# Maaz77/Head-Pose-Estimation-Model

Hardware: AMD Instinct MI355X
Metric: images/sec (train+infer) on 96×96 feature maps; yaw/pitch/roll MAE vs ref (higher is better)
Workload: dtype fp32; 1 GPU; Model-96 create_model(num_filters=360, dropout=0, l2=0.1) training, legacy Adam lr 2.8e-4, 96x96 feature maps (configs[3] per GPU: 512 images per rank); global_batch=512, per_gpu_batch=512, positions_per_image=9216, channels=96, parallelism=dp1

## Files before the change

### head-pose-estimation-model_amd/csrc/hpe_mlp2.hip

```cpp
#include <hip/hip_runtime.h>
#include <stdint.h>
#include <stdlib.h>

#include "hpe_common.h"
#include "hpe_dev.h"

#ifdef MLP2_BIG
#define MLP2_NS mlp2_big
#else
#define MLP2_NS mlp2_small
#endif
#define MLP2_BIG_ROWS (1 << 15)
namespace MLP2_NS {

#define MLP2_MAXW 12
#ifndef MLP2_BAR1_SKIP
#define MLP2_BAR1_SKIP 1
#endif
#ifndef MLP2_W88
#define MLP2_W88 2
#endif
#define MLP2_XS 100
#define MLP2_XF (32 * MLP2_XS)
#define MLP2_LAB 128
#define MLP2_RED 32
#define MLP2_FS 104
#define MLP2_TS 40
#define MLP2_A1W (15 * 68 + 64)
#define MLP2_PRE_HALVES (3 * 32 * MLP2_FS + 2 * 3 * 96 * MLP2_TS)

struct E2 {
  int act, drop;
  uint32_t thr;
  float keep;
};

struct TileImg {
  int img0, rem0, P;
  template <bool P32 = false>
  __device__ __forceinline__ int of(int r) const {
    const int t = rem0 + r;
    if (P32) return img0 + (t >= P ? 1 : 0);
    return img0 + (P >= 32 ? (t >= P ? 1 : 0) : (P == 1 ? t : t / P));
  }
  __device__ __forceinline__ void advance(int dq, int dr) {
    img0 += dq;
    rem0 += dr;
    if (rem0 >= P) { rem0 -= P; ++img0; }
  }
};

__device__ __forceinline__ float e_fwd(const E2& e, uint64_t seed, int64_t img, int ch, float z) {
  float a = act_f(e.act, z);
  if (e.drop >= 0) a = drop_hash(seed, e.drop, (uint64_t)img, ch) >= e.thr ? a / e.keep : 0.f;
  return a;
}

__device__ __forceinline__ float e_bwd(const E2& e, uint64_t seed, int64_t img, int ch, float g, float val) {
  if (e.drop >= 0) {
    if (drop_hash(seed, e.drop, (uint64_t)img, ch) < e.thr) return 0.f;
    g = g / e.keep;
    val = val * e.keep;
  }
  return e.act == ACT_LINEAR ? g : g * act_grad(e.act, val, 0.f);
}

__device__ __forceinline__ void stage_tile(const Args& args, float* xs, float* lab, int64_t row0,
                                           const TileImg& ti, int wave, int NCB, int lane, int Cin,
                                           bool labels, int XS = MLP2_XS) {
  const int64_t rem = args.nrows - 1 - row0;
  const int last = rem < 31 ? (int)rem : 31;
  const int P = args.P;
  const int q = Cin >> 2;
  if (!args.idx && P >= 32) {
    if (labels && wave == 0) {
#pragma unroll
      for (int pc = 0; pc < 2; ++pc) {
        const int slot = pc * 64 + lane;
        const int r = min(slot >> 2, last), j = min(slot & 3, 2);
        glds4(args.ytrue + (int64_t)ti.of(r) * 3 + j, lds_addr(lab + pc * 64));
      }
    }
    for (int r = wave; r < 32; r += NCB) {
      const int64_t srow = row0 + min(r, last);
      if (lane < q) glds16(args.x + srow * Cin + 4 * lane, lds_addr(xs + r * XS));
    }
    return;
  }
  const int lr = min(lane & 31, last);
  const int limg = ti.of(lr);
  const int lpos = (int)(row0 + lr - (int64_t)limg * P);
  const int lsrc = args.idx ? args.idx[limg] : limg;
  __builtin_amdgcn_s_waitcnt(0x0F70);
  if (labels && wave == 0) {
#pragma unroll
    for (int pc = 0; pc < 2; ++pc) {
      const int slot = pc * 64 + lane;
      const int r = min(slot >> 2, last), j = min(slot & 3, 2);
      const int64_t src = __shfl(lsrc, r, 64);
      glds4(args.ytrue + src * 3 + j, lds_addr(lab + pc * 64));
    }
  }
  for (int r = wave; r < 32; r += NCB) {
    const int rr = min(r, last);
    const int64_t srow = (int64_t)__builtin_amdgcn_readlane(lsrc, rr) * P +
                         __builtin_amdgcn_readlane(lpos, rr);
    if (lane < q) glds16(args.x + srow * Cin + 4 * lane, lds_addr(xs + r * XS));
  }
}

__device__ __forceinline__ int lane_now() {
  int l;
  asm volatile("v_mbcnt_lo_u32_b32 %0, -1, 0\n\tv_mbcnt_hi_u32_b32 %0, -1, %0" : "=v"(l));
  return l;
}

__device__ __forceinline__ void stage_contig(const Args& args, float* xs, float* lab, const float* tp,
                                             int64_t row0, const TileImg& ti, int wave, int NCB, int Cin,
                                             bool labels) {
  const int lane = lane_now();
  const int64_t rem = args.nrows - 1 - row0;
  const int last = rem < 31 ? (int)rem : 31;
  if (labels && wave == 0) {
    const float* yp = args.ytrue + (int64_t)ti.img0 * 3;
#pragma unroll
    for (int pc = 0; pc < 2; ++pc) {
      const int slot = pc * 64 + lane;
      const int r = min(slot >> 2, last), j = min(slot & 3, 2);
      glds4(yp + (ti.rem0 + r >= ti.P ? 3 + j : j), lds_addr(lab + pc * 64));
    }
  }
  const int q = Cin >> 2;
  for (int r = wave; r < 32; r += NCB)
    if (lane < q) glds16(tp + min(r, last) * Cin + 4 * lane, lds_addr(xs + r * MLP2_XS));
}

typedef _Float16 h4 __attribute__((ext_vector_type(4)));

__device__ __forceinline__ void split_d4(f32x4 v, h4& ch, h4& cl, h4& h) {
  const f32x4 s = v * SPLIT_C;
  ch = __builtin_convertvector(s, h4);
  cl = __builtin_convertvector(s - __builtin_convertvector(ch, f32x4), h4);
  h = __builtin_convertvector(v, h4);
}
__device__ __forceinline__ constexpr int a1_row(int g) { return 68 * (g ^ ((g >> 1) & 4)); }
#define MLP2_X_LIMIT (65520.f / SPLIT_C)
template <int KH>
__device__ __forceinline__ bool presplit_tile(const float* xs, _Float16* xf, _Float16* xt, int tid, int NT) {
  bool out = false;
  for (int i = tid; i < 32 * 24; i += NT) {
    const int r = i / 24, rem = i - r * 24, h = rem >= 12 ? 1 : 0, m0 = 4 * (rem - 12 * h);
    const f32x4 v = m0 < KH ? *(const f32x4*)(xs + r * MLP2_XS + KH * h + m0) : f32x4{0.f, 0.f, 0.f, 0.f};
    out |= !(fabsf(v.x) < MLP2_X_LIMIT) | !(fabsf(v.y) < MLP2_X_LIMIT) | !(fabsf(v.z) < MLP2_X_LIMIT) |
           !(fabsf(v.w) < MLP2_X_LIMIT);
    h4 ch, cl, hh;
    split_d4(v, ch, cl, hh);
    _Float16* d = xf + r * MLP2_FS + 48 * h + m0;
    *(h4*)(d) = ch;
    *(h4*)(d + 32 * MLP2_FS) = cl;
    *(h4*)(d + 64 * MLP2_FS) = hh;
  }
  for (int i = tid; i < 96 * 8; i += NT) {
    const int rg = i / 96, k = i - rg * 96, r = 4 * rg;
    const f32x4 v = {xs[r * MLP2_XS + k], xs[(r + 1) * MLP2_XS + k], xs[(r + 2) * MLP2_XS + k],
                     xs[(r + 3) * MLP2_XS + k]};
    const int p = (r & ~12) | ((r & 4) << 1) | ((r & 8) >> 1);
    h4 ch, cl, hh;
    split_d4(v, ch, cl, hh);
    _Float16* d = xt + k * MLP2_TS + p;
    *(h4*)(d) = ch;
    *(h4*)(d + 96 * MLP2_TS) = cl;
    *(h4*)(d + 192 * MLP2_TS) = hh;
  }
  return out;
}

template <int KH, int ACT1, bool DROP, int NWM, bool SPLIT, bool CONTIG = false>
__global__ void __launch_bounds__(NWM * 64) __attribute__((amdgpu_waves_per_eu(NWM == MLP2_MAXW || ACT1 < 0 ? 1 : MLP2_W88, 8))) mlp2_kernel(Args args) {
  static_assert(!CONTIG || (SPLIT && NWM == MLP2_MAXW), "CONTIG is an instantiation of the pre-split kernel");
  if (!SPLIT && args.guard && __hip_atomic_load(args.guard, __ATOMIC_RELAXED, __HIP_MEMORY_SCOPE_AGENT) != args.epoch) return;
#ifdef MLP2_STAMPS
  const uint64_t rt0 = __builtin_amdgcn_s_memrealtime();
#endif
  extern __shared__ __attribute__((aligned(16))) float lds[];
  constexpr int NKB = (2 * KH + 31) / 32;
  constexpr int T = 32;
  constexpr bool PRE = SPLIT && NWM == MLP2_MAXW;
  constexpr int NXB = PRE ? 1 : 2;
  constexpr bool LEAN = PRE && ACT1 >= 0;
  constexpr bool PAD1 = true;
  constexpr int A1S = MLP2_A1W;
  constexpr int HS = NWM == MLP2_MAXW ? 4 : 3;
  const int* prog = args.prog;
  const int* o = prog + prog[H_OPS_OFF];
  const int mode = prog[H_MODE];
  const bool train = mode == MODE_TRAIN;
  const int Cin = o[O_K], F = o[O_N], NCB = o[O_MODE];
  const int wave = __builtin_amdgcn_readfirstlane(threadIdx.x >> 6);
  const int lane = threadIdx.x & 63, half = lane >> 5, l32 = lane & 31;
  const int NT = blockDim.x;
  const int n = wave * 32 + l32;
  const bool nok = n < F;
  const int NPR = NWM == MLP2_MAXW ? MLP2_MAXW : NCB;
  float* xbuf = lds;
  float* lbuf = xbuf + NXB * MLP2_XF;
  float* part = lbuf + 2 * MLP2_LAB;
  float* dz2 = part + NPR * T * 4;
  float* a1s = dz2 + T * 4;
  float* w2t = a1s + NCB * A1S;
  float* b2t = w2t + NCB * 128;
  float* hacc = b2t + 4;
  float* red = hacc + NCB * 64 * HS;
  float* colt = red + MLP2_RED;
  _Float16* xfb = (_Float16*)(colt + NCB * 128);
  _Float16* xtb = xfb + 3 * 32 * MLP2_FS;

  E2 e1 = {o[O_EACT], o[O_EDROP], (uint32_t)o[O_ETHR], __int_as_float(o[O_EKEEP])};
  E2 e2 = {o[O_AUX2], o[O_TBASE], (uint32_t)o[O_TCOUNT], __int_as_float(o[O_F0])};
  const float inv_keep1 = 1.f / e1.keep;
  const float* W1 = args.params + o[O_W];
  const float* W2 = args.params + o[O_AUX0];

  const int64_t nrows = args.nrows;
  const int64_t ntiles = (nrows + T - 1) / T;
  const int P = args.P;
  const bool labels = mode != MODE_FWD;
  const int S = gridDim.x * T, dq = S / P, dr = S - dq * P;
  TileImg ti;
  ti.P = P;
  ti.img0 = (int)(blockIdx.x * T / P);
  ti.rem0 = (int)(blockIdx.x * T - ti.img0 * P);
  const float* xnext = CONTIG ? args.x + (int64_t)blockIdx.x * T * Cin : nullptr;
  const int64_t xstep = CONTIG ? (int64_t)gridDim.x * T * Cin : 0;
  if (blockIdx.x < ntiles) {
    if constexpr (CONTIG) stage_contig(args, xbuf, lbuf, xnext, (int64_t)blockIdx.x * T, ti, wave, NCB, Cin, labels);
    else stage_tile(args, xbuf, lbuf, (int64_t)blockIdx.x * T, ti, wave, NCB, lane, Cin, labels);
  }
  xnext += xstep;
  const int nc = min(n, F - 1);
  const float w2a = W2[nc * 3], w2b = W2[nc * 3 + 1], w2c = W2[nc * 3 + 2];
  const int o_bias = __builtin_amdgcn_readfirstlane(o[O_BIAS]), o_aux1 = __builtin_amdgcn_readfirstlane(o[O_AUX1]);
  const float b1r = args.params[max(o_bias, 0) + nc];
  float w2r[2];
#pragma unroll
  for (int t = 0; t < 2; ++t) {
    const int i = threadIdx.x + t * NT, nn = i >> 2, j = i & 3;
    w2r[t] = W2[min(nn, F - 1) * 3 + min(j, 2)];
  }
  const float b2r = args.params[max(o_aux1, 0) + min((int)threadIdx.x & 3, 2)];

  float wreg[SPLIT ? 1 : KH];
  SplitW wsp[SPLIT ? 6 : 1];
  float inv1 = 1.f, s2 = 1.f;
  bool wbad = false;
  if constexpr (SPLIT) {
    f32x8 v[6];
#pragma unroll
    for (int s = 0; s < 6; ++s) {
#pragma unroll
      for (int j = 0; j < 8; ++j) {
        const int k = half * KH + 8 * s + j;
        v[s][j] = 8 * s + j < KH ? W1[(size_t)min(k, Cin - 1) * F + nc] : 0.f;
      }
    }
    __builtin_amdgcn_sched_barrier(0);
    float mx = 0.f;
#pragma unroll
    for (int s = 0; s < 6; ++s) {
#pragma unroll
      for (int j = 0; j < 8; ++j) {
        const int k = half * KH + 8 * s + j;
        v[s][j] = (k < Cin && nok) ? v[s][j] : 0.f;
        mx = fmaxf(mx, fabsf(v[s][j]));
      }
    }
    mx = fmaxf(mx, __shfl_xor(mx, 32, 64));
    const float s1 = pow2_scale(mx, 13);
    inv1 = SPLIT_INV_C / s1;
#pragma unroll
    for (int s = 0; s < 6; ++s) {
      const f32x8 vs = v[s] * s1;
      wsp[s] = split_w8(vs);
      if (PRE) {
#pragma unroll
        for (int j = 0; j < 8; ++j) wbad |= !(fabsf(vs[j]) < 65520.f);
      }
    }
    s2 = pow2_scale(nok ? fmaxf(fmaxf(fabsf(w2a), fabsf(w2b)), fabsf(w2c)) : 0.f, 2);
  } else {
#pragma unroll
    for (int m = 0; m < KH; ++m) {
      const int k = half * KH + m;
      const float wv = W1[(size_t)min(k, Cin - 1) * F + nc];
      wreg[m] = (k < Cin && nok) ? wv : 0.f;
    }
  }
  bool bad = PRE && wbad && blockIdx.x < ntiles;
  {
    const float b1 = (nok && o_bias >= 0) ? b1r : 0.f;
    if (half == 0) *(f32x4*)(colt + n * 4) = f32x4{inv1, b1, s2, 0.f};
  }
#pragma unroll
  for (int t = 0; t < 2; ++t) {
    const int i = threadIdx.x + t * NT, nn = i >> 2, j = i & 3;
    if (i < NCB * 128) w2t[i] = (nn < F && j < 3) ? w2r[t] : 0.f;
  }
  if (threadIdx.x < 4) b2t[threadIdx.x] = (threadIdx.x < 3 && o_aux1 >= 0) ? b2r : 0.f;
  for (int i = threadIdx.x; i < NT * HS; i += NT) hacc[i] = 0.f;

  f32x16 dw[NKB];
#pragma unroll
  for (int s = 0; s < NKB; ++s) dw[s] = f32x16{};
  float dw2[3] = {0.f, 0.f, 0.f};
  float db1 = 0.f;

  const int NT3 = (NT / 3) * 3;

  for (int i = threadIdx.x; i < NXB * 32 * 16; i += NT) {
    const int r = i >> 4, c = Cin + (i & 15);
    if (c < 96) xbuf[r * MLP2_XS + c] = 0.f;
  }
  for (int i = NCB * T * 4 + threadIdx.x; i < NPR * T * 4; i += NT) part[i] = 0.f;
  __syncthreads();
  if constexpr (PRE) {
    asm volatile("s_waitcnt vmcnt(0)" ::: "memory");
    bar_lds();
    const bool xbad = presplit_tile<KH>(xbuf, xfb, xtb, threadIdx.x, NT);
    bad |= xbad && blockIdx.x < ntiles;
  }
  int buf = 0;
#ifdef MLP2_STAMPS
  uint32_t ph[9] = {};
  uint64_t tprev = __builtin_amdgcn_s_memtime();
  const uint64_t rt1 = __builtin_amdgcn_s_memrealtime();
#define STAMP(i) do { const uint64_t t_ = __builtin_amdgcn_s_memtime(); ph[i] += (uint32_t)(t_ - tprev); tprev = t_; } while (0)
#else
#define STAMP(i) do {} while (0)
#endif
  for (int tile = blockIdx.x; tile < (int)ntiles; tile += gridDim.x, buf ^= 1, ti.advance(dq, dr)) {
    const int tlane = PRE ? lane_now() : lane, thalf = tlane >> 5, tl32 = tlane & 31;
    const int tcol = wave * 32 + tl32;
    const bool tok = tcol < F;
    const int64_t row0 = (int64_t)tile * T;
    const float* xs = xbuf + (PRE ? 0 : buf) * MLP2_XF;
    const float* lab = lbuf + buf * MLP2_LAB;
    if constexpr (!PRE) asm volatile("s_waitcnt vmcnt(0)" ::: "memory");
    STAMP(0);
    if (!(MLP2_BAR1_SKIP && PRE && NCB >= 4 && tile != (int)blockIdx.x)) bar_lds();
    STAMP(1);
    if (tile + gridDim.x < ntiles) {
      TileImg tn = ti;
      tn.advance(dq, dr);
      if constexpr (CONTIG) {
        stage_contig(args, xbuf, lbuf + (buf ^ 1) * MLP2_LAB, xnext, (int64_t)(tile + gridDim.x) * T, tn,
                     wave, NCB, Cin, labels);
        xnext += xstep;
      } else {
        stage_tile(args, xbuf + (PRE ? 0 : (buf ^ 1)) * MLP2_XF, lbuf + (buf ^ 1) * MLP2_LAB,
                   (int64_t)(tile + gridDim.x) * T, tn, wave, NCB, tlane, Cin, labels);
      }
    }

    STAMP(2);
    uint32_t dmask = 0;
    {
      const float* ap = xs + tl32 * MLP2_XS + thalf * KH;
      f32x16 acc = {};
      if constexpr (PRE) {
        const _Float16* fp = xfb + tl32 * MLP2_FS + 48 * thalf;
        auto frag = [&](int s) {
          return SplitD{*(const h8*)(fp + 8 * s), *(const h8*)(fp + 32 * MLP2_FS + 8 * s),
                        *(const h8*)(fp + 64 * MLP2_FS + 8 * s)};
        };
        SplitD xd = frag(0);
#pragma unroll
        for (int s = 0; s < 6; ++s) {
          SplitD xn = xd;
          if (s + 1 < 6) xn = frag(s + 1);
          __builtin_amdgcn_sched_barrier(0);
          acc = mfma3_dw(xd, wsp[s], acc);
          xd = xn;
        }
        STAMP(3);
      } else if constexpr (SPLIT) {
#pragma unroll
        for (int s = 0; s < 6; ++s) {
          const f32x4 a0 = *(const f32x4*)(ap + 8 * s), a1 = *(const f32x4*)(ap + 8 * s + 4);
          acc = mfma3_dw(split_d8(f32x8{a0.x, a0.y, a0.z, a0.w, a1.x, a1.y, a1.z, a1.w}), wsp[s], acc);
          __builtin_amdgcn_sched_barrier(0);
        }
        bad |= !(fabsf(sum16(acc)) <= 3.0e38f);
      } else {
        f32x4 an = *(const f32x4*)(ap);
#pragma unroll
        for (int m = 0; m < KH; m += 4) {
          const f32x4 a = an;
          if (m + 4 < KH) an = *(const f32x4*)(ap + m + 4);
          acc = __builtin_amdgcn_mfma_f32_32x32x2f32(a.x, wreg[m + 0], acc, 0, 0, 0);
          acc = __builtin_amdgcn_mfma_f32_32x32x2f32(a.y, wreg[m + 1], acc, 0, 0, 0);
          acc = __builtin_amdgcn_mfma_f32_32x32x2f32(a.z, wreg[m + 2], acc, 0, 0, 0);
          acc = __builtin_amdgcn_mfma_f32_32x32x2f32(a.w, wreg[m + 3], acc, 0, 0, 0);
          __builtin_amdgcn_sched_barrier(0);
        }
      }
      if (DROP) {
        if (CONTIG || P >= 32) {
          const bool k0 = drop_hash(args.seed, e1.drop, (uint64_t)(ti.img0 + args.img_off), tcol) >= e1.thr;
          const bool k1 = drop_hash(args.seed, e1.drop, (uint64_t)(ti.img0 + 1 + args.img_off), tcol) >= e1.thr;
#pragma unroll
          for (int g = 0; g < 16; ++g) {
            const int r = (g & 3) + 8 * (g >> 2) + 4 * thalf;
            dmask |= (ti.rem0 + r >= P ? k1 : k0) ? (1u << g) : 0u;
          }
        } else {
#pragma unroll
          for (int g = 0; g < 16; ++g) {
            const int r = (g & 3) + 8 * (g >> 2) + 4 * thalf;
            dmask |= drop_hash(args.seed, e1.drop, (uint64_t)(ti.of(r) + args.img_off), tcol) >= e1.thr
                         ? (1u << g) : 0u;
          }
        }
      }
      const f32x4 cs = *(const f32x4*)(colt + tcol * 4);
#pragma unroll
      for (int g = 0; g < 16; ++g) {
        float z = act1_f<ACT1, SPLIT>(e1.act, SPLIT ? fmaf(acc[g], cs.x, cs.y) : acc[g] + cs.y);
        if (DROP) z = (dmask >> g) & 1u ? z * inv_keep1 : 0.f;
        acc[g] = LEAN || tok ? z : 0.f;
      }
#pragma unroll
      for (int g = 0; g < 16; ++g) a1s[wave * A1S + (PAD1 ? a1_row(g) : 64 * g) + tlane] = acc[g];
      __builtin_amdgcn_fence(__ATOMIC_RELEASE, "wavefront");
      __builtin_amdgcn_wave_barrier();
      __builtin_amdgcn_fence(__ATOMIC_ACQUIRE, "wavefront");
      {
        const int r = tl32, hh = (r >> 2) & 1, gr = (r & 3) + 4 * (r >> 3);
        const float* ar = a1s + wave * A1S + (PAD1 ? a1_row(gr) : 64 * gr) + hh * 32 + 16 * thalf;
        const float* wr = w2t + (wave * 32 + 16 * thalf) * 4;
        float s0 = 0.f, s1 = 0.f, s2 = 0.f;
#pragma unroll
        for (int i = 0; i < 16; i += 4) {
          const f32x4 av = *(const f32x4*)(ar + i);
#pragma unroll
          for (int e = 0; e < 4; ++e) {
            const f32x4 w = *(const f32x4*)(wr + (i + e) * 4);
            s0 = fmaf(av[e], w.x, s0);
            s1 = fmaf(av[e], w.y, s1);
            s2 = fmaf(av[e], w.z, s2);
          }
        }
        s0 += __shfl_xor(s0, 32, 64);
        s1 += __shfl_xor(s1, 32, 64);
        s2 += __shfl_xor(s2, 32, 64);
        if (thalf == 0) *(f32x4*)(part + (wave * T + r) * 4) = f32x4{s0, s1, s2, 0.f};
      }
    }
    STAMP(4);
    const bool early = PRE && NCB >= 4;
    if (early) asm volatile("s_waitcnt vmcnt(0)" ::: "memory");
    bar_lds();
    STAMP(5);
    if constexpr (PRE) {
      if (early && wave >= 2 && tile + gridDim.x < ntiles)
        bad |= presplit_tile<KH>(xbuf, xfb, xtb + (buf ^ 1) * 3 * 96 * MLP2_TS, threadIdx.x - 128, NT - 128);
    }

    auto head_item = [&](int it) {
      const int r = it / 3, j = it - r * 3;
      const int64_t R = row0 + r;
      float z = b2t[j];
      float pv[MLP2_MAXW];
#pragma unroll
      for (int w = 0; w < MLP2_MAXW; ++w) pv[w] = NWM == MLP2_MAXW || w < NCB ? part[(w * T + r) * 4 + j] : 0.f;
      float lv = 0.f, ha0 = 0.f, ha1 = 0.f, ha2 = 0.f;
      if (mode != MODE_FWD) {
        lv = lab[r * 4 + j];
        ha0 = hacc[threadIdx.x * HS + 0];
        ha1 = hacc[threadIdx.x * HS + 1];
        ha2 = hacc[threadIdx.x * HS + 2];
      }
#pragma unroll
      for (int w = 0; w < MLP2_MAXW; ++w) z += pv[w];
      const bool d2 = ACT1 < 0 || __builtin_expect(e2.drop >= 0, 0);
      int64_t img = 0;
      bool k2 = true;
      if (d2) {
        img = ti.of<CONTIG>(r) + args.img_off;
        if (ACT1 >= 0) k2 = drop_hash(args.seed, e2.drop, (uint64_t)img, j) >= e2.thr;
      }
      const float p = ACT1 >= 0 ? (d2 ? (k2 ? z / e2.keep : 0.f) : z) : e_fwd(e2, args.seed, img, j, z);
      if (mode == MODE_FWD) {
        if (R < nrows) args.y[R * 3 + j] = p;
      } else {
        float g = 0.f;
        if (R < nrows) {
          const float err = p - lv;
          ha0 = fmaf(err, err, ha0);
          ha1 += fabsf(err);
          g = SPLIT ? 2.f * err : 2.f * err * args.inv_count;
        }
        if (train) {
          g = ACT1 >= 0 ? (d2 ? (k2 ? g / e2.keep : 0.f) : g) : e_bwd(e2, args.seed, img, j, g, p);
          dz2[r * 4 + j] = g;
          ha2 += g;
        }
        hacc[threadIdx.x * HS + 0] = ha0;
        hacc[threadIdx.x * HS + 1] = ha1;
        hacc[threadIdx.x * HS + 2] = ha2;
      }
    };
    if constexpr (NWM == MLP2_MAXW) {
      if (threadIdx.x < T * 3) head_item(threadIdx.x);
    } else {
      for (int it = threadIdx.x; it < T * 3 && threadIdx.x < NT3; it += NT3) head_item(it);
    }
    STAMP(6);
    if constexpr (PRE) {
      asm volatile("s_waitcnt vmcnt(0)" ::: "memory");
      bar_lds();
      STAMP(7);
      if (!early && tile + gridDim.x < ntiles) {
        bad |= presplit_tile<KH>(xbuf, xfb, xtb + (buf ^ 1) * 3 * 96 * MLP2_TS, threadIdx.x, NT);
      }
      if (!train) continue;
    } else {
      if (!train) continue;
      bar_lds();
    }

    STAMP(8);
    {
      const f32x4 w2r = *(const f32x4*)(w2t + tcol * 4);
      const float s2 = colt[tcol * 4 + 2];
      const f32x4 w2v = PRE ? f32x4{w2r.x * s2, w2r.y * s2, w2r.z * s2, 0.f} : w2r;
      auto dz_of = [&](int g) {
        const int r = (g & 3) + 8 * (g >> 2) + 4 * thalf;
        const f32x4 d = *(const f32x4*)(dz2 + r * 4);
        const float a = a1s[wave * A1S + (PAD1 ? a1_row(g) : 64 * g) + tlane];
        const float da = PRE ? fmaf(d.z, w2v.z, fmaf(d.x, w2v.x, d.y * w2v.y))
                             : d.x * w2v.x + d.y * w2v.y + d.z * w2v.z;
        float gz, av = a;
        if (DROP) {
          gz = (dmask >> g) & 1u ? da * inv_keep1 : 0.f;
          av = a * e1.keep;
        } else {
          gz = da;
        }
        {
#pragma clang fp contract(off)
          gz = LEAN || tok ? gz * act1_g<ACT1>(e1.act, av) : 0.f;
          db1 += gz;
        }
        dw2[0] = fmaf(a, d.x, dw2[0]);
        dw2[1] = fmaf(a, d.y, dw2[1]);
        dw2[2] = fmaf(a, d.z, dw2[2]);
        return gz;
      };
      if constexpr (PRE) {
        const _Float16* th = xtb + buf * 3 * 96 * MLP2_TS + tl32 * MLP2_TS + 8 * thalf;
        f32x8 dv0, dv1;
#pragma unroll
        for (int j = 0; j < 8; ++j) dv0[j] = dz_of(j);
        const SplitW d0 = split_w8(dv0);
        __builtin_amdgcn_sched_barrier(0);
#pragma unroll
        for (int kb = 0; kb < NKB; ++kb) {
          const _Float16* q = th + kb * 32 * MLP2_TS;
          dw[kb] = mfma3_dw(SplitD{*(const h8*)(q), *(const h8*)(q + 96 * MLP2_TS), *(const h8*)(q + 192 * MLP2_TS)}, d0, dw[kb]);
        }
#pragma unroll
        for (int j = 0; j < 8; ++j) dv1[j] = dz_of(8 + j);
        __builtin_amdgcn_sched_barrier(0);
        const SplitW d1 = split_w8(dv1);
#pragma unroll
        for (int kb = 0; kb < NKB; ++kb) {
          const _Float16* q = th + 16 + kb * 32 * MLP2_TS;
          dw[kb] = mfma3_dw(SplitD{*(const h8*)(q), *(const h8*)(q + 96 * MLP2_TS), *(const h8*)(q + 192 * MLP2_TS)}, d1, dw[kb]);
        }
      } else if constexpr (SPLIT) {
#pragma unroll
        for (int s = 0; s < 2; ++s) {
          f32x8 dv;
#pragma unroll
          for (int j = 0; j < 8; ++j) {
            dv[j] = dz_of(8 * s + j);
            if ((j & 3) == 3) __builtin_amdgcn_sched_barrier(0);
          }
          const SplitW dsp = split_w8(dv * s2);
#pragma unroll
          for (int kb = 0; kb < NKB; ++kb) {
            const float* xp = xs + (4 * thalf) * MLP2_XS + kb * 32 + tl32;
            f32x8 xv;
#pragma unroll
            for (int j = 0; j < 8; ++j) xv[j] = xp[(16 * s + 8 * (j >> 2) + (j & 3)) * MLP2_XS];
            dw[kb] = mfma3_dw(split_d8(xv), dsp, dw[kb]);
            __builtin_amdgcn_sched_barrier(0);
          }
        }
      } else {
        float dz1[16];
#pragma unroll
        for (int g = 0; g < 16; ++g) {
          dz1[g] = dz_of(g);
          if ((g & 3) == 3) __builtin_amdgcn_sched_barrier(0);
        }
#pragma unroll
        for (int kb = 0; kb < NKB; ++kb) {
          const float* xp = xs + (4 * thalf) * MLP2_XS + kb * 32 + tl32;
          f32x16 acc = dw[kb];
          auto xat = [&](int g) { return xp[((g & 3) + 8 * (g >> 2)) * MLP2_XS]; };
          float x0 = xat(0), x1 = xat(1);
#pragma unroll
          for (int g = 0; g < 16; ++g) {
            const float xv = x0;
            x0 = x1;
            if (g + 2 < 16) x1 = xat(g + 2);
            acc = __builtin_amdgcn_mfma_f32_32x32x2f32(xv, dz1[g], acc, 0, 0, 0);
            __builtin_amdgcn_sched_barrier(0);
          }
          dw[kb] = acc;
        }
      }
    }
  }

#ifdef MLP2_STAMPS
  const uint64_t rt2 = __builtin_amdgcn_s_memrealtime();
  uint64_t rtA = 0, rtB = 0;
  if (PRE && blockIdx.x == 0 && lane == 0 && (wave == 0 || wave == 5))
    printf("STAMP w%d bwd+tail %u bar1 %u stage %u fwdmfma %u act+part %u bar2 %u head %u bar3 %u presplit %u\n", wave,
           ph[0], ph[1], ph[2], ph[3], ph[4], ph[5], ph[6], ph[7], ph[8]);
#endif
  const int flane = PRE ? lane_now() : lane, fhalf = flane >> 5;
  const int fcol = wave * 32 + (flane & 31);
  const bool fok = fcol < F;
  if (mode == MODE_FWD) {
    if (SPLIT && bad) __hip_atomic_store(args.guard, args.epoch, __ATOMIC_RELAXED, __HIP_MEMORY_SCOPE_AGENT);
    return;
  }
  const int slab = prog[H_SLAB];
  const int npt = prog[H_NPARAMS_TRAIN];
  float* ws = args.ws + (size_t)blockIdx.x * slab;
  const float sc = SPLIT ? args.inv_count : 1.f;
  const int oW = __builtin_amdgcn_readfirstlane(o[O_W]), oB = __builtin_amdgcn_readfirstlane(o[O_BIAS]);
  const int oA0 = __builtin_amdgcn_readfirstlane(o[O_AUX0]), oA1 = __builtin_amdgcn_readfirstlane(o[O_AUX1]);
  __syncthreads();
  const float s2f = colt[fcol * 4 + 2];
  if (train) {
    const float scw = SPLIT ? sc * (SPLIT_INV_C / s2f) : sc;
    float chk = 0.f;
#pragma unroll
    for (int kb = 0; kb < NKB; ++kb) {
      if (SPLIT) chk += sum16(dw[kb]);
#pragma unroll
      for (int g = 0; g < 16; ++g) {
        const int k = kb * 32 + (g & 3) + 8 * (g >> 2) + 4 * fhalf;
        if (k < Cin && fok) ws[oW + (size_t)k * F + fcol] = dw[kb][g] * scw;
      }
    }
    if (SPLIT) bad |= (!LEAN || fok) && !(fabsf(chk) <= 3.0e38f);
    const float tb = (db1 + __shfl_xor(db1, 32, 64)) * (PRE ? 1.f / s2f : 1.f);
    float t2[3];
#pragma unroll
    for (int j = 0; j < 3; ++j) t2[j] = dw2[j] + __shfl_xor(dw2[j], 32, 64);
    if (fhalf == 0 && fok) {
      if (oB >= 0) ws[oB + fcol] = tb * sc;
#pragma unroll
      for (int j = 0; j < 3; ++j) ws[oA0 + fcol * 3 + j] = t2[j] * sc;
    }
#ifdef MLP2_STAMPS
    rtA = __builtin_amdgcn_s_memrealtime();
#endif
    if (oA1 >= 0) {
      for (int j = wave; j < 3; j += NT >> 6) {
        float s = 0.f;
        for (int i = j + 3 * flane; i < NT3; i += 192) s += hacc[i * HS + 2];
        s = wave_sum(s);
        if (flane == 0) ws[oA1 + j] = s * sc;
      }
    }
#ifdef MLP2_STAMPS
    rtB = __builtin_amdgcn_s_memrealtime();
#endif
    __syncthreads();
  }
#ifdef MLP2_STAMPS
  const uint64_t rtC = __builtin_amdgcn_s_memrealtime();
#endif
  if (SPLIT && bad) __hip_atomic_store(args.guard, args.epoch, __ATOMIC_RELAXED, __HIP_MEMORY_SCOPE_AGENT);
  const float a = wave_sum(hacc[threadIdx.x * HS + 0]), b = wave_sum(hacc[threadIdx.x * HS + 1]);
  if (flane == 0) { red[wave] = a; red[MLP2_MAXW + wave] = b; }
  __syncthreads();
  if (threadIdx.x == 0) {
    float s0 = 0.f, s1 = 0.f;
    const int nw = NT >> 6;
    for (int w = 0; w < nw; ++w) { s0 += red[w]; s1 += red[MLP2_MAXW + w]; }
    ws[npt] = s0;
    ws[npt + 1] = s1;
  }
#ifdef MLP2_STAMPS
  if (PRE && threadIdx.x == 0) {
    const uint64_t rt3 = __builtin_amdgcn_s_memrealtime();
    printf("RT wg %d t0 %llu pro %llu loop %llu flush %llu wstore %llu db2 %llu sync %llu tail %llu\n", (int)blockIdx.x, (unsigned long long)rt0,
           (unsigned long long)(rt1 - rt0), (unsigned long long)(rt2 - rt1), (unsigned long long)(rt3 - rt2),
           (unsigned long long)(rtA - rt2), (unsigned long long)(rtB - rtA), (unsigned long long)(rtC - rtB), (unsigned long long)(rt3 - rtC));
  }
#endif
}

#ifdef MLP2_BIG
#define MLP2R_NU 2
#define MLP2R_LDS_FLOATS (2 * MLP2_XF + 2 * MLP2_LAB + MLP2R_NU * MLP2_A1W + 32 * 4 + MLP2R_NU * 128 + 4)

template <int KH, int ACT1, bool DROP>
__global__ void __launch_bounds__(64) __attribute__((amdgpu_waves_per_eu(1, 1))) mlp2r_kernel(Args args) {
  extern __shared__ __attribute__((aligned(16))) float lds[];
  constexpr int NU = MLP2R_NU;
  constexpr int NKB = (2 * KH + 31) / 32;
  constexpr int T = 32;
  constexpr int XS = KH == 44 ? 88 : MLP2_XS;
  const int* prog = args.prog;
  const int* o = prog + prog[H_OPS_OFF];
  const int Cin = o[O_K], F = o[O_N];
  const int lane = threadIdx.x, half = lane >> 5, l32 = lane & 31;
  float* xbuf = lds;
  float* lbuf = xbuf + 2 * MLP2_XF;
  float* a1p = lbuf + 2 * MLP2_LAB;
  float* dz2 = a1p + NU * MLP2_A1W;
  float* w2t = dz2 + 32 * 4;
  float* b2t = w2t + NU * 128;
  const E2 e1 = {o[O_EACT], o[O_EDROP], (uint32_t)o[O_ETHR], __int_as_float(o[O_EKEEP])};
  const E2 e2 = {o[O_AUX2], o[O_TBASE], (uint32_t)o[O_TCOUNT], __int_as_float(o[O_F0])};
  const float inv_keep1 = 1.f / e1.keep, inv_keep2 = 1.f / e2.keep;
  const float* W1 = args.params + o[O_W];
  const float* W2 = args.params + o[O_AUX0];
  const int o_bias = __builtin_amdgcn_readfirstlane(o[O_BIAS]), o_aux1 = __builtin_amdgcn_readfirstlane(o[O_AUX1]);

  const int64_t nrows = args.nrows;
  const int64_t ntiles = (nrows + T - 1) / T;
  const int P = args.P;
  const int S = gridDim.x * T, dq = S / P, dr = S - dq * P;
  TileImg ti;
  ti.P = P;
  ti.img0 = (int)(blockIdx.x * T / P);
  ti.rem0 = (int)(blockIdx.x * T - ti.img0 * P);
  auto stage = [&](float* xd, float* ld, int64_t r0, const TileImg& t) {
    if (XS == 88 && !args.idx && P >= 32 && r0 + T <= nrows && Cin == 88) {
#pragma unroll
      for (int pc = 0; pc < 2; ++pc) {
        const int slot = pc * 64 + lane;
        glds4(args.ytrue + (int64_t)t.of(slot >> 2) * 3 + min(slot & 3, 2), lds_addr(ld + pc * 64));
      }
#pragma unroll
      for (int i = 0; i < 11; ++i) glds16(args.x + r0 * 88 + 256 * i + 4 * lane, lds_addr(xd + 256 * i));
    } else {
      stage_tile(args, xd, ld, r0, t, 0, 1, lane, Cin, true, XS);
    }
  };
  if (blockIdx.x < ntiles) stage(xbuf, lbuf, (int64_t)blockIdx.x * T, ti);

  SplitW wsp[NU][6];
  float inv1[NU], b1v[NU], s2[NU], nm[NU];
  f32x4 w2v[NU];
  bool nok[NU];
  {
    f32x8 v[NU][6];
    float w2r[NU][3], b1r[NU];
#pragma unroll
    for (int u = 0; u < NU; ++u) {
      const int n = 32 * u + l32, nc = min(n, F - 1);
      nok[u] = n < F;
      nm[u] = nok[u] ? 1.f : 0.f;
#pragma unroll
      for (int j = 0; j < 3; ++j) w2r[u][j] = W2[nc * 3 + j];
      b1r[u] = args.params[max(o_bias, 0) + nc];
#pragma unroll
      for (int s = 0; s < 6; ++s) {
#pragma unroll
        for (int j = 0; j < 8; ++j) {
          const int k = half * KH + 8 * s + j;
          v[u][s][j] = 8 * s + j < KH ? W1[(size_t)min(k, Cin - 1) * F + nc] : 0.f;
        }
      }
    }
    const float b2r = args.params[max(o_aux1, 0) + min(lane & 3, 2)];
    __builtin_amdgcn_sched_barrier(0);
#pragma unroll
    for (int u = 0; u < NU; ++u) {
      float mx = 0.f;
#pragma unroll
      for (int s = 0; s < 6; ++s) {
#pragma unroll
        for (int j = 0; j < 8; ++j) {
          const int k = half * KH + 8 * s + j;
          v[u][s][j] = (k < Cin && nok[u]) ? v[u][s][j] : 0.f;
          mx = fmaxf(mx, fabsf(v[u][s][j]));
        }
      }
      mx = fmaxf(mx, __shfl_xor(mx, 32, 64));
      const float s1 = pow2_scale(mx, 13);
      inv1[u] = SPLIT_INV_C / s1;
#pragma unroll
      for (int s = 0; s < 6; ++s) wsp[u][s] = split_w8(v[u][s] * s1);
      w2v[u] = nok[u] ? f32x4{w2r[u][0], w2r[u][1], w2r[u][2], 0.f} : f32x4{0.f, 0.f, 0.f, 0.f};
      s2[u] = pow2_scale(nok[u] ? fmaxf(fmaxf(fabsf(w2r[u][0]), fabsf(w2r[u][1])), fabsf(w2r[u][2])) : 0.f, 2);
      b1v[u] = (nok[u] && o_bias >= 0) ? b1r[u] : 0.f;
      if (half == 0) *(f32x4*)(w2t + (32 * u + l32) * 4) = w2v[u];
    }
    if (lane < 4) b2t[lane] = (lane < 3 && o_aux1 >= 0) ? b2r : 0.f;
  }
  if (XS == 88) {
    for (int i = lane; i < 2 * (MLP2_XF - 32 * 88); i += 64)
      xbuf[(i >= MLP2_XF - 32 * 88 ? MLP2_XF : 0) + 32 * 88 + i % (MLP2_XF - 32 * 88)] = 0.f;
  } else {
    for (int i = lane; i < 2 * 32 * 16; i += 64) {
      const int r = i >> 4, c = Cin + (i & 15);
      if (c < 96) xbuf[r * MLP2_XS + c] = 0.f;
    }
  }

  f32x16 dw[NU][NKB];
#pragma unroll
  for (int u = 0; u < NU; ++u)
#pragma unroll
    for (int kb = 0; kb < NKB; ++kb) dw[u][kb] = f32x16{};
  float dw2[NU][3], db1[NU];
#pragma unroll
  for (int u = 0; u < NU; ++u) { dw2[u][0] = dw2[u][1] = dw2[u][2] = 0.f; db1[u] = 0.f; }
  float sse = 0.f, sae = 0.f, db2[3] = {0.f, 0.f, 0.f};
  bool bad = false;

  int buf = 0;
#ifdef MLP2R_STAMPS
  uint32_t ph[7] = {};
  uint64_t tprev = __builtin_amdgcn_s_memtime();
#define RSTAMP(i) do { const uint64_t t_ = __builtin_amdgcn_s_memtime(); ph[i] += (uint32_t)(t_ - tprev); tprev = t_; } while (0)
#else
#define RSTAMP(i) do {} while (0)
#endif
  for (int64_t tile = blockIdx.x; tile < ntiles; tile += gridDim.x, buf ^= 1, ti.advance(dq, dr)) {
    const int64_t row0 = tile * T;
    RSTAMP(0);
    asm volatile("s_waitcnt vmcnt(0)" ::: "memory");
    if (tile + gridDim.x < ntiles) {
      TileImg tn = ti;
      tn.advance(dq, dr);
      stage(xbuf + (buf ^ 1) * MLP2_XF, lbuf + (buf ^ 1) * MLP2_LAB, (tile + gridDim.x) * T, tn);
    }
    const float* xs = xbuf + buf * MLP2_XF;
    const float* lab = lbuf + buf * MLP2_LAB;
    RSTAMP(1);

    f32x16 acc[NU];
#pragma unroll
    for (int u = 0; u < NU; ++u) acc[u] = f32x16{};
    {
      const float* ap = xs + l32 * XS + half * KH;
      f32x4 xa[12];
#pragma unroll
      for (int s = 0; s < 12; ++s) xa[s] = *(const f32x4*)(ap + 4 * s);
#pragma unroll
      for (int s = 0; s < 6; ++s) {
        const f32x4 a0 = xa[2 * s], a1 = xa[2 * s + 1];
        const SplitD xd = split_d8(f32x8{a0.x, a0.y, a0.z, a0.w, a1.x, a1.y, a1.z, a1.w});
#pragma unroll
        for (int u = 0; u < NU; ++u) acc[u] = mfma3_dw(xd, wsp[u][s], acc[u]);
      }
    }
    RSTAMP(2);
    uint32_t dmask[NU];
#pragma unroll
    for (int u = 0; u < NU; ++u) {
      bad |= !(fabsf(sum16(acc[u])) <= 3.0e38f);
      const int n = 32 * u + l32;
      dmask[u] = 0u;
      if (DROP) {
        if (P >= 32) {
          const bool k0 = drop_hash(args.seed, e1.drop, (uint64_t)(ti.img0 + args.img_off), n) >= e1.thr;
          const bool k1 = drop_hash(args.seed, e1.drop, (uint64_t)(ti.img0 + 1 + args.img_off), n) >= e1.thr;
#pragma unroll
          for (int g = 0; g < 16; ++g) {
            const int r = (g & 3) + 8 * (g >> 2) + 4 * half;
            dmask[u] |= (ti.rem0 + r >= P ? k1 : k0) ? (1u << g) : 0u;
          }
        } else {
#pragma unroll
          for (int g = 0; g < 16; ++g) {
            const int r = (g & 3) + 8 * (g >> 2) + 4 * half;
            dmask[u] |= drop_hash(args.seed, e1.drop, (uint64_t)(ti.of(r) + args.img_off), n) >= e1.thr ? (1u << g) : 0u;
          }
        }
      }
#pragma unroll
      for (int g = 0; g < 16; ++g) {
        const float km = DROP ? ((dmask[u] >> g) & 1u ? inv_keep1 : 0.f) : 1.f;
        acc[u][g] = act1_f<ACT1>(e1.act, fmaf(acc[u][g], inv1[u], b1v[u])) * km * nm[u];
        a1p[u * MLP2_A1W + a1_row(g) + lane] = acc[u][g];
      }
    }
    __builtin_amdgcn_fence(__ATOMIC_RELEASE, "wavefront");
    __builtin_amdgcn_wave_barrier();
    __builtin_amdgcn_fence(__ATOMIC_ACQUIRE, "wavefront");

    RSTAMP(3);
    {
      const int r = l32, hh = (r >> 2) & 1, gr = (r & 3) + 4 * (r >> 3);
      const f32x4 lv = *(const f32x4*)(lab + r * 4);
      float h0 = 0.f, h1 = 0.f, h2 = 0.f;
#pragma unroll
      for (int u = 0; u < NU; ++u) {
        const float* ar = a1p + u * MLP2_A1W + a1_row(gr) + hh * 32 + 16 * half;
        const float* wr = w2t + (32 * u + 16 * half) * 4;
        f32x4 av[4], wv[16];
#pragma unroll
        for (int i = 0; i < 4; ++i) av[i] = *(const f32x4*)(ar + 4 * i);
#pragma unroll
        for (int i = 0; i < 16; ++i) wv[i] = *(const f32x4*)(wr + 4 * i);
#pragma unroll
        for (int i = 0; i < 16; ++i) {
          h0 = fmaf(av[i >> 2][i & 3], wv[i].x, h0);
          h1 = fmaf(av[i >> 2][i & 3], wv[i].y, h1);
          h2 = fmaf(av[i >> 2][i & 3], wv[i].z, h2);
        }
      }
      h0 += __shfl_xor(h0, 32, 64);
      h1 += __shfl_xor(h1, 32, 64);
      h2 += __shfl_xor(h2, 32, 64);
      if (half == 0) {
        const bool valid = row0 + r < nrows;
        const bool d2 = __builtin_expect(e2.drop >= 0, 0);
        const int64_t img = d2 ? ti.of(r) + args.img_off : 0;
        const float zs[3] = {b2t[0] + h0, b2t[1] + h1, b2t[2] + h2};
        float gs[3];
#pragma unroll
        for (int j = 0; j < 3; ++j) {
          const bool k2 = d2 ? drop_hash(args.seed, e2.drop, (uint64_t)img, j) >= e2.thr : true;
          const float kk = d2 ? (k2 ? inv_keep2 : 0.f) : 1.f;
          const float p = zs[j] * kk;
          float g = 0.f;
          if (valid) {
            const float err = p - lv[j];
            sse = fmaf(err, err, sse);
            sae += fabsf(err);
            g = 2.f * err;
          }
          g *= kk;
          db2[j] += g;
          gs[j] = g;
        }
        *(f32x4*)(dz2 + r * 4) = f32x4{gs[0], gs[1], gs[2], 0.f};
      }
    }
    __builtin_amdgcn_fence(__ATOMIC_RELEASE, "wavefront");
    __builtin_amdgcn_wave_barrier();
    __builtin_amdgcn_fence(__ATOMIC_ACQUIRE, "wavefront");

    RSTAMP(4);
    f32x4 dzr[16];
#pragma unroll
    for (int g = 0; g < 16; ++g) dzr[g] = *(const f32x4*)(dz2 + ((g & 3) + 8 * (g >> 2) + 4 * half) * 4);
    f32x8 xtr[2][NKB];
#pragma unroll
    for (int s = 0; s < 2; ++s)
#pragma unroll
      for (int kb = 0; kb < NKB; ++kb)
#pragma unroll
        for (int j = 0; j < 8; ++j)
          xtr[s][kb][j] = xs[(4 * half + 16 * s + 8 * (j >> 2) + (j & 3)) * XS + kb * 32 + l32];
#pragma unroll
    for (int s = 0; s < 2; ++s) {
      f32x8 dv[NU];
#pragma unroll
      for (int j = 0; j < 8; ++j) {
        const int g = 8 * s + j;
        const f32x4 d = dzr[g];
#pragma unroll
        for (int u = 0; u < NU; ++u) {
          const float a = acc[u][g];
          const float da = d.x * w2v[u].x + d.y * w2v[u].y + d.z * w2v[u].z;
          const float km = DROP ? ((dmask[u] >> g) & 1u ? inv_keep1 : 0.f) : 1.f;
          const float gz = da * km * act1_g<ACT1>(e1.act, DROP ? a * e1.keep : a) * nm[u];
          dw2[u][0] = fmaf(a, d.x, dw2[u][0]);
          dw2[u][1] = fmaf(a, d.y, dw2[u][1]);
          dw2[u][2] = fmaf(a, d.z, dw2[u][2]);
          db1[u] += gz;
          dv[u][j] = gz;
        }
      }
      SplitW dsp[NU];
#pragma unroll
      for (int u = 0; u < NU; ++u) dsp[u] = split_w8(dv[u] * s2[u]);
#pragma unroll
      for (int kb = 0; kb < NKB; ++kb) {
        const SplitD xd = split_d8(xtr[s][kb]);
#pragma unroll
        for (int u = 0; u < NU; ++u) dw[u][kb] = mfma3_dw(xd, dsp[u], dw[u][kb]);
      }
      if (s == 0) RSTAMP(5);
    }
    RSTAMP(6);
  }
#ifdef MLP2R_STAMPS
  if (blockIdx.x < 2 && lane == 0)
    printf("RSTAMP wg %d top %u stage %u fwd %u act %u head %u bwd0 %u bwd1 %u\n", (int)blockIdx.x, ph[0], ph[1], ph[2], ph[3], ph[4], ph[5], ph[6]);
#endif

  const int slab = prog[H_SLAB];
  const int npt = prog[H_NPARAMS_TRAIN];
  float* ws = args.ws + (size_t)blockIdx.x * slab;
  const float sc = args.inv_count;
  const int oW = __builtin_amdgcn_readfirstlane(o[O_W]), oA0 = __builtin_amdgcn_readfirstlane(o[O_AUX0]);
  float chk = 0.f;
#pragma unroll
  for (int u = 0; u < NU; ++u) {
    const int n = 32 * u + l32;
    const float scw = sc * (SPLIT_INV_C / s2[u]);
#pragma unroll
    for (int kb = 0; kb < NKB; ++kb) {
      chk += sum16(dw[u][kb]);
#pragma unroll
      for (int g = 0; g < 16; ++g) {
        const int k = kb * 32 + (g & 3) + 8 * (g >> 2) + 4 * half;
        if (k < Cin && nok[u]) ws[oW + (size_t)k * F + n] = dw[u][kb][g] * scw;
      }
    }
    const float tb = db1[u] + __shfl_xor(db1[u], 32, 64);
    float t2[3];
#pragma unroll
    for (int j = 0; j < 3; ++j) t2[j] = dw2[u][j] + __shfl_xor(dw2[u][j], 32, 64);
    if (half == 0 && nok[u]) {
      if (o_bias >= 0) ws[o_bias + n] = tb * sc;
#pragma unroll
      for (int j = 0; j < 3; ++j) ws[oA0 + n * 3 + j] = t2[j] * sc;
    }
  }
  bad |= !(fabsf(chk) <= 3.0e38f);
#pragma unroll
  for (int j = 0; j < 3; ++j) {
    const float t = wave_sum(db2[j]);
    if (lane == 0 && o_aux1 >= 0) ws[o_aux1 + j] = t * sc;
  }
  if (bad) __hip_atomic_store(args.guard, args.epoch, __ATOMIC_RELAXED, __HIP_MEMORY_SCOPE_AGENT);
  const float ta = wave_sum(sse), tb = wave_sum(sae);
  if (lane == 0) {
    ws[npt] = ta;
    ws[npt + 1] = tb;
  }
}
#endif

typedef void (*mlp2_fn)(Args);

template <int KH, bool DROP, int NWM, bool SPLIT, bool CONTIG = false>
static mlp2_fn pick_act(int act, int act2) {
  if (act2 != ACT_LINEAR) return mlp2_kernel<KH, -1, DROP, NWM, SPLIT, CONTIG>;
  if (act == ACT_TANH) return mlp2_kernel<KH, ACT_TANH, DROP, NWM, SPLIT, CONTIG>;
  if (act == ACT_SOFTSIGN) return mlp2_kernel<KH, ACT_SOFTSIGN, DROP, NWM, SPLIT, CONTIG>;
  return mlp2_kernel<KH, -1, DROP, NWM, SPLIT, CONTIG>;
}

template <bool DROP, bool SPLIT>
static mlp2_fn pick_d(int kh, int act, int act2, int ncb, bool contig) {
  if (ncb <= 4) {
    if (kh == 44) return pick_act<44, DROP, 4, SPLIT>(act, act2);
    if (kh == 48) return pick_act<48, DROP, 4, SPLIT>(act, act2);
  }
  if constexpr (SPLIT) {
    if (contig && kh == 44) return pick_act<44, DROP, MLP2_MAXW, SPLIT, true>(act, act2);
    if (contig && kh == 48) return pick_act<48, DROP, MLP2_MAXW, SPLIT, true>(act, act2);
  }
  if (kh == 44) return pick_act<44, DROP, MLP2_MAXW, SPLIT>(act, act2);
  if (kh == 48) return pick_act<48, DROP, MLP2_MAXW, SPLIT>(act, act2);
  return nullptr;
}

static mlp2_fn pick(const int* w, bool split = false, bool contig = false) {
  const int* o = w + w[H_OPS_OFF];
  const int kh = ((o[O_K] + 7) & ~7) / 2, act = o[O_EACT], act2 = o[O_AUX2];
  if (split)
    return o[O_EDROP] >= 0 ? pick_d<true, true>(kh, act, act2, o[O_MODE], contig) : pick_d<false, true>(kh, act, act2, o[O_MODE], contig);
  return o[O_EDROP] >= 0 ? pick_d<true, false>(kh, act, act2, o[O_MODE], false) : pick_d<false, false>(kh, act, act2, o[O_MODE], false);
}

static void geom(const int* w, int& kh, int& rbw, int& ncb, int& lds_bytes, int& act, int& drop) {
  const int* o = w + w[H_OPS_OFF];
  act = o[O_EACT];
  drop = o[O_EDROP];
  const int cin = o[O_K];
  const int cp = (cin + 7) & ~7;
  kh = cp / 2;
  rbw = o[O_FLAGS];
  ncb = o[O_MODE];
  const int T = 32;
  const int npr = ncb > 4 ? MLP2_MAXW : ncb;
  const int rest = 2 * MLP2_LAB + npr * T * 4 + T * 4 + ncb * MLP2_A1W + ncb * 128 + 4 + ncb * 64 * (ncb > 4 ? 4 : 3) + MLP2_RED + ncb * 128;
  lds_bytes = (2 * MLP2_XF + rest) * 4;
  const int pre = (MLP2_XF + rest) * 4 + MLP2_PRE_HALVES * 2;
  if (ncb > 4 && pre > lds_bytes) lds_bytes = pre;
}

static int lds_split(const int* w) {
  int kh, rbw, ncb, lds, act, drop;
  geom(w, kh, rbw, ncb, lds, act, drop);
  return lds;
}

static int launch_k(mlp2_fn k, int nw, int lds, const Args& a, int grid, hipStream_t s) {
  hipFuncSetAttribute((const void*)k, hipFuncAttributeMaxDynamicSharedMemorySize, lds);
  hipLaunchKernelGGL(k, dim3(grid), dim3(nw * 64), lds, s, a);
  return hipGetLastError() == hipSuccess ? 0 : 2;
}

static bool split_only() {
  const char* e = getenv("HPE_SPLIT_ONLY");
  return e && e[0] == '1';
}

#ifdef MLP2_BIG
template <int KH>
static mlp2_fn pick_r_act(int act, bool drop) {
  if (act == ACT_TANH) return drop ? mlp2r_kernel<KH, ACT_TANH, true> : mlp2r_kernel<KH, ACT_TANH, false>;
  if (act == ACT_SOFTSIGN) return drop ? mlp2r_kernel<KH, ACT_SOFTSIGN, true> : mlp2r_kernel<KH, ACT_SOFTSIGN, false>;
  return nullptr;
}
static mlp2_fn pick_r(const int* w) {
  const char* e = getenv("HPE_MLP2_ROWS");
  if ((e && e[0] == '0') || w[H_MODE] != MODE_TRAIN) return nullptr;
  const int* o = w + w[H_OPS_OFF];
  if (o[O_MODE] > MLP2R_NU || o[O_N] > 32 * MLP2R_NU || o[O_AUX2] != ACT_LINEAR) return nullptr;
  const int kh = ((o[O_K] + 7) & ~7) / 2;
  if (kh == 44 && o[O_K] == 88) return pick_r_act<44>(o[O_EACT], o[O_EDROP] >= 0);
  if (kh == 48) return pick_r_act<48>(o[O_EACT], o[O_EDROP] >= 0);
  return nullptr;
}
#else
static mlp2_fn pick_r(const int*) { return nullptr; }
#define MLP2R_LDS_FLOATS 0
#endif

static int launch_pair(const int* w, const Args& a, int grid, hipStream_t s) {
  int kh, rbw, ncb, lds, act, drop;
  geom(w, kh, rbw, ncb, lds, act, drop);
  if (hpe_exact_fp32() || !a.guard) {
    Args e = a;
    e.guard = nullptr;
    const int tv = hpe_tev_begin(s);
    const int rc = launch_k(pick(w), ncb, lds, e, grid, s);
    hpe_tev_end(s, tv);
    return rc;
  }
  const mlp2_fn kr = pick_r(w);
  const int tv = hpe_tev_begin(s);
  const bool contig = a.idx == nullptr && a.P >= 32;
  const int rc = kr ? launch_k(kr, 1, MLP2R_LDS_FLOATS * 4, a, grid, s) : launch_k(pick(w, true, contig), ncb, lds_split(w), a, grid, s);
  hpe_tev_end(s, tv);
  if (rc) return rc;
  if (split_only()) return 0;
  if (a.x_bound > 0.f && a.x_bound < SPLIT_DATA_RANGE) return 0;
  return launch_k(pick(w), ncb, lds, a, grid, s);
}

static int per_cu_of(mlp2_fn k, int ncb, int lds) {
  hipFuncAttributes attr;
  int per_cu = 1;
  if (hipFuncGetAttributes(&attr, (const void*)k) == hipSuccess) {
    const int vg = ((attr.numRegs + 7) / 8) * 8;
    const int waves_simd = vg > 0 ? (512 / vg > 8 ? 8 : 512 / vg) : 8;
    per_cu = (4 * waves_simd) / ncb;
  }
  const int by_lds = (160 * 1024) / lds;
  if (per_cu > by_lds) per_cu = by_lds;
  return per_cu < 1 ? 1 : per_cu;
}

static int cap_per_cu(const int* w) {
  int kh, rbw, ncb, lds, act, drop;
  geom(w, kh, rbw, ncb, lds, act, drop);
  int cap = per_cu_of(pick(w), ncb, lds);
  const int b = per_cu_of(pick(w, true), ncb, lds_split(w)), bc = per_cu_of(pick(w, true, true), ncb, lds_split(w));
  cap = b < cap ? b : cap;
  cap = bc < cap ? bc : cap;
  const mlp2_fn kr = pick_r(w);
  if (kr) {
    const int c = per_cu_of(kr, 1, MLP2R_LDS_FLOATS * 4);
    cap = c < cap ? c : cap;
  }
  return cap;
}
}

#ifdef MLP2_BIG
int mlp2_launch_big(const int* w, const Args& a, int grid, hipStream_t s) {
  return MLP2_NS::launch_pair(w, a, grid, s);
}
int mlp2_per_cu_big(const int* w) { return MLP2_NS::cap_per_cu(w); }
#else
using namespace MLP2_NS;
int mlp2_launch_big(const int* w, const Args& a, int grid, hipStream_t s);
int mlp2_per_cu_big(const int* w);

int mlp2_supported(const int* w) {
  int kh, rbw, ncb, lds, act, drop;
  geom(w, kh, rbw, ncb, lds, act, drop);
  const int* o = w + w[H_OPS_OFF];
  return pick(w) != nullptr && rbw == 1 && ncb >= 1 && ncb <= MLP2_MAXW &&
         o[O_AUX3] == 3 && (o[O_K] & 3) == 0 && o[O_K] <= 96 && lds <= 160 * 1024;
}

int mlp2_grid_cap(const int* w, int n_cu) {
  const int a = MLP2_NS::cap_per_cu(w), b = mlp2_per_cu_big(w);
  return n_cu * (a < b ? a : b);
}

int mlp2_launch(const int* w, const Args& a, int grid, hipStream_t s) {
  if (a.nrows >= MLP2_BIG_ROWS) return mlp2_launch_big(w, a, grid, s);
  return launch_pair(w, a, grid, s);
}
#endif
```

Before: 181,700 images/sec.

## Drop transposed presplit copy; read weight-grad operands via ds_read_tr16 transpose loads

Removes the separate transposed fp16 split buffer (xt) and instead reads the dW operands straight from the row-major split buffer with the LDS transpose-read instruction ds_read_tr16_b64. The row-major split buffer is now double-buffered per tile, the presplit runs at 8-wide granularity, and the early presplit/barrier-skip path is applied unconditionally for PRE instead of only when NCB>=4. This removes half the presplit writes and LDS footprint, at the cost of depending on transpose-load lane mapping correctness and changed scheduling for smaller NCB configurations.

```diff
diff --git a/head-pose-estimation-model_amd/csrc/hpe_mlp2.hip b/head-pose-estimation-model_amd/csrc/hpe_mlp2.hip
--- a/head-pose-estimation-model_amd/csrc/hpe_mlp2.hip
+++ b/head-pose-estimation-model_amd/csrc/hpe_mlp2.hip
@@ -25,9 +25,9 @@
 #define MLP2_LAB 128
 #define MLP2_RED 32
 #define MLP2_FS 104
-#define MLP2_TS 40
+#define MLP2_IMG (3 * 32 * MLP2_FS)
 #define MLP2_A1W (15 * 68 + 64)
-#define MLP2_PRE_HALVES (3 * 32 * MLP2_FS + 2 * 3 * 96 * MLP2_TS)
+#define MLP2_PRE_HALVES (2 * MLP2_IMG)
 
 struct E2 {
   int act, drop;
@@ -137,40 +137,37 @@
 
 typedef _Float16 h4 __attribute__((ext_vector_type(4)));
 
-__device__ __forceinline__ void split_d4(f32x4 v, h4& ch, h4& cl, h4& h) {
-  const f32x4 s = v * SPLIT_C;
-  ch = __builtin_convertvector(s, h4);
-  cl = __builtin_convertvector(s - __builtin_convertvector(ch, f32x4), h4);
-  h = __builtin_convertvector(v, h4);
+typedef __fp16 fp16x4 __attribute__((__vector_size__(4 * sizeof(__fp16))));
+
+template <int KH>
+__device__ __forceinline__ int img_pos(int c) {
+  if (KH == 48) return c;
+  return c < KH ? c : min(c + 48 - KH, 92);
+}
+__device__ __forceinline__ h8 tr_read8(const _Float16* p) {
+  typedef __attribute__((address_space(3))) fp16x4* lp;
+  const fp16x4 a = __builtin_amdgcn_ds_read_tr16_b64_v4f16((lp)(p));
+  const fp16x4 b = __builtin_amdgcn_ds_read_tr16_b64_v4f16((lp)(p + 8 * MLP2_FS));
+  return __builtin_shufflevector(__builtin_bit_cast(h4, a), __builtin_bit_cast(h4, b), 0, 1, 2, 3, 4, 5, 6, 7);
 }
 __device__ __forceinline__ constexpr int a1_row(int g) { return 68 * (g ^ ((g >> 1) & 4)); }
 #define MLP2_X_LIMIT (65520.f / SPLIT_C)
 template <int KH>
-__device__ __forceinline__ bool presplit_tile(const float* xs, _Float16* xf, _Float16* xt, int tid, int NT) {
+__device__ __forceinline__ bool presplit_tile(const float* xs, _Float16* xf, int tid, int NT) {
   bool out = false;
-  for (int i = tid; i < 32 * 24; i += NT) {
-    const int r = i / 24, rem = i - r * 24, h = rem >= 12 ? 1 : 0, m0 = 4 * (rem - 12 * h);
-    const f32x4 v = m0 < KH ? *(const f32x4*)(xs + r * MLP2_XS + KH * h + m0) : f32x4{0.f, 0.f, 0.f, 0.f};
-    out |= !(fabsf(v.x) < MLP2_X_LIMIT) | !(fabsf(v.y) < MLP2_X_LIMIT) | !(fabsf(v.z) < MLP2_X_LIMIT) |
-           !(fabsf(v.w) < MLP2_X_LIMIT);
-    h4 ch, cl, hh;
-    split_d4(v, ch, cl, hh);
+  for (int i = tid; i < 32 * 12; i += NT) {
+    const int r = i / 12, rem = i - r * 12, h = rem >= 6 ? 1 : 0, m0 = 8 * (rem - 6 * h);
+    const float* s = xs + r * MLP2_XS + KH * h + m0;
+    const f32x4 z = {0.f, 0.f, 0.f, 0.f};
+    const f32x4 a = *(const f32x4*)(s), b = m0 + 4 < KH ? *(const f32x4*)(s + 4) : z;
+    const f32x8 v = {a.x, a.y, a.z, a.w, b.x, b.y, b.z, b.w};
+#pragma unroll
+    for (int j = 0; j < 8; ++j) out |= !(fabsf(v[j]) < MLP2_X_LIMIT);
+    const SplitD d8 = split_d8(v);
     _Float16* d = xf + r * MLP2_FS + 48 * h + m0;
-    *(h4*)(d) = ch;
-    *(h4*)(d + 32 * MLP2_FS) = cl;
-    *(h4*)(d + 64 * MLP2_FS) = hh;
-  }
-  for (int i = tid; i < 96 * 8; i += NT) {
-    const int rg = i / 96, k = i - rg * 96, r = 4 * rg;
-    const f32x4 v = {xs[r * MLP2_XS + k], xs[(r + 1) * MLP2_XS + k], xs[(r + 2) * MLP2_XS + k],
-                     xs[(r + 3) * MLP2_XS + k]};
-    const int p = (r & ~12) | ((r & 4) << 1) | ((r & 8) >> 1);
-    h4 ch, cl, hh;
-    split_d4(v, ch, cl, hh);
-    _Float16* d = xt + k * MLP2_TS + p;
-    *(h4*)(d) = ch;
-    *(h4*)(d + 96 * MLP2_TS) = cl;
-    *(h4*)(d + 192 * MLP2_TS) = hh;
+    *(h8*)(d) = d8.ch;
+    *(h8*)(d + 32 * MLP2_FS) = d8.cl;
+    *(h8*)(d + 64 * MLP2_FS) = d8.h;
   }
   return out;
 }
@@ -213,7 +210,6 @@
   float* red = hacc + NCB * 64 * HS;
   float* colt = red + MLP2_RED;
   _Float16* xfb = (_Float16*)(colt + NCB * 128);
-  _Float16* xtb = xfb + 3 * 32 * MLP2_FS;
 
   E2 e1 = {o[O_EACT], o[O_EDROP], (uint32_t)o[O_ETHR], __int_as_float(o[O_EKEEP])};
   E2 e2 = {o[O_AUX2], o[O_TBASE], (uint32_t)o[O_TCOUNT], __int_as_float(o[O_F0])};
@@ -325,7 +321,7 @@
   if constexpr (PRE) {
     asm volatile("s_waitcnt vmcnt(0)" ::: "memory");
     bar_lds();
-    const bool xbad = presplit_tile<KH>(xbuf, xfb, xtb, threadIdx.x, NT);
+    const bool xbad = presplit_tile<KH>(xbuf, xfb, threadIdx.x, NT);
     bad |= xbad && blockIdx.x < ntiles;
   }
   int buf = 0;
@@ -346,7 +342,7 @@
     const float* lab = lbuf + buf * MLP2_LAB;
     if constexpr (!PRE) asm volatile("s_waitcnt vmcnt(0)" ::: "memory");
     STAMP(0);
-    if (!(MLP2_BAR1_SKIP && PRE && NCB >= 4 && tile != (int)blockIdx.x)) bar_lds();
+    if (!(MLP2_BAR1_SKIP && PRE && tile != (int)blockIdx.x)) bar_lds();
     STAMP(1);
     if (tile + gridDim.x < ntiles) {
       TileImg tn = ti;
@@ -367,7 +363,7 @@
       const float* ap = xs + tl32 * MLP2_XS + thalf * KH;
       f32x16 acc = {};
       if constexpr (PRE) {
-        const _Float16* fp = xfb + tl32 * MLP2_FS + 48 * thalf;
+        const _Float16* fp = xfb + buf * MLP2_IMG + tl32 * MLP2_FS + 48 * thalf;
         auto frag = [&](int s) {
           return SplitD{*(const h8*)(fp + 8 * s), *(const h8*)(fp + 32 * MLP2_FS + 8 * s),
                         *(const h8*)(fp + 64 * MLP2_FS + 8 * s)};
@@ -456,13 +452,12 @@
       }
     }
     STAMP(4);
-    const bool early = PRE && NCB >= 4;
-    if (early) asm volatile("s_waitcnt vmcnt(0)" ::: "memory");
+    if constexpr (PRE) asm volatile("s_waitcnt vmcnt(0)" ::: "memory");
     bar_lds();
     STAMP(5);
     if constexpr (PRE) {
-      if (early && wave >= 2 && tile + gridDim.x < ntiles)
-        bad |= presplit_tile<KH>(xbuf, xfb, xtb + (buf ^ 1) * 3 * 96 * MLP2_TS, threadIdx.x - 128, NT - 128);
+      if (wave >= 2 && tile + gridDim.x < ntiles)
+        bad |= presplit_tile<KH>(xbuf, xfb + (buf ^ 1) * MLP2_IMG, threadIdx.x - 128, NT - 128);
     }
 
     auto head_item = [&](int it) {
@@ -519,9 +514,6 @@
       asm volatile("s_waitcnt vmcnt(0)" ::: "memory");
       bar_lds();
       STAMP(7);
-      if (!early && tile + gridDim.x < ntiles) {
-        bad |= presplit_tile<KH>(xbuf, xfb, xtb + (buf ^ 1) * 3 * 96 * MLP2_TS, threadIdx.x, NT);
-      }
       if (!train) continue;
     } else {
       if (!train) continue;
@@ -557,7 +549,12 @@
         return gz;
       };
       if constexpr (PRE) {
-        const _Float16* th = xtb + buf * 3 * 96 * MLP2_TS + tl32 * MLP2_TS + 8 * thalf;
+        const int tc = (tl32 & 16) + 4 * (tl32 & 3);
+        const _Float16* th = xfb + buf * MLP2_IMG + (4 * thalf + ((tl32 >> 2) & 3)) * MLP2_FS;
+        auto xt_of = [&](int s, int kb) {
+          const _Float16* q = th + 16 * s * MLP2_FS + img_pos<KH>(32 * kb + tc);
+          return SplitD{tr_read8(q), tr_read8(q + 32 * MLP2_FS), tr_read8(q + 64 * MLP2_FS)};
+        };
         f32x8 dv0, dv1;
 #pragma unroll
         for (int j = 0; j < 8; ++j) dv0[j] = dz_of(j);
@@ -565,18 +562,15 @@
         __builtin_amdgcn_sched_barrier(0);
 #pragma unroll
         for (int kb = 0; kb < NKB; ++kb) {
-          const _Float16* q = th + kb * 32 * MLP2_TS;
-          dw[kb] = mfma3_dw(SplitD{*(const h8*)(q), *(const h8*)(q + 96 * MLP2_TS), *(const h8*)(q + 192 * MLP2_TS)}, d0, dw[kb]);
+          dw[kb] = mfma3_dw(xt_of(0, kb), d0, dw[kb]);
+          if (kb == 0) __builtin_amdgcn_sched_barrier(0);
         }
 #pragma unroll
         for (int j = 0; j < 8; ++j) dv1[j] = dz_of(8 + j);
         __builtin_amdgcn_sched_barrier(0);
         const SplitW d1 = split_w8(dv1);
 #pragma unroll
-        for (int kb = 0; kb < NKB; ++kb) {
-          const _Float16* q = th + 16 + kb * 32 * MLP2_TS;
-          dw[kb] = mfma3_dw(SplitD{*(const h8*)(q), *(const h8*)(q + 96 * MLP2_TS), *(const h8*)(q + 192 * MLP2_TS)}, d1, dw[kb]);
-        }
+        for (int kb = 0; kb < NKB; ++kb) dw[kb] = mfma3_dw(xt_of(1, kb), d1, dw[kb]);
       } else if constexpr (SPLIT) {
 #pragma unroll
         for (int s = 0; s < 2; ++s) {
```

Result: faster. 187,100 images/sec (median of 6 runs) (+2.9%).
